# rishihahs/pupperv3-mjx

Hardware: AMD Instinct MI355X
Metric: env-steps/sec at N_envs=4096/GPU, 1/2/4/8 MI355X; qpos rel-err vs mj_step (higher is better)
Workload: dtype f32

## Files before the change

### pupperv3-mjx_amd/csrc/pp3_env.hip

```cpp
#include <hip/hip_runtime.h>

#include <float.h>
#include <math.h>
#include <stddef.h>
#include <stdio.h>
#include <stdlib.h>
#include <string.h>

#include <string>
#include <algorithm>
#include <vector>

#include "pp3_device.h"
#include "pp3_diag.h"
#include "pp3_mlp.h"

namespace pp3 {

constexpr int HW = 32;
typedef __attribute__((address_space(4))) const DevModel GModel;
typedef __attribute__((address_space(4))) const float GFloat;
constexpr int HMAX = 16;
constexpr int OBS_MOVE = (PP3_OBS_DIM * (HMAX - 1) + HW - 1) / HW;
template <int HCAP, int LAGCAP>
// ... 580 lines not shown
  if (r >= c) { r -= c; m >>= 8; pos += 8; }
  c = __popc(m & 0xFu);
  if (r >= c) { r -= c; m >>= 4; pos += 4; }
  c = __popc(m & 0x3u);
  if (r >= c) { r -= c; m >>= 2; pos += 2; }
  return pos + (r >= (int)(m & 1u) ? 1 : 0);
}

template <int NC, int NWV = 1, bool CULL = false>
__device__ __forceinline__ int collision(Shared<NC>& s, const DevModel& m, int l, int h, const PairLoad& pre,
                                         float* ccache = nullptr) {
  int nhit = 0;
  const TerrainRef tr{m.terrain, m.nbox};
  auto run = [&](int p, const PairLoad& pl) {
    float dist = 0, pos[3], nrm[3];
    v4f pc0;
    const bool hit = narrow<NC, NWV>(s, tr, pl, dist, pos, nrm, pc0) && p >= 0;
    const uint32_t mask = hballot(hit, h);
    const int slot = nhit + __popc(mask & ((1u << l) - 1u));
    if (hit) {
      if (slot < NC) store_contact(s, pc0, slot, p, dist, pos, nrm);
      if (slot < NHIT) { s.x.a.hit_dist[slot] = dist; s.x.a.hit_pair[slot] = p; }
    }
    nhit += __popc(mask);
  };
  if (!CULL || !m.cull_on) {
    for (int base = 0; base < m.npair; base += HW) {
      const int p = base + l;
      float dist = 0, pos[3], nrm[3];
      v4f pc0;
      const PairLoad pl = base == 0 ? pre : load_pair(m, p < m.npair ? p : 0);
      const bool hit = narrow<NC, NWV>(s, tr, pl, dist, pos, nrm, pc0) && (p < m.npair);
      const uint32_t mask = hballot(hit, h);
      const int slot = nhit + __popc(mask & ((1u << l) - 1u));
      if (hit) {
        if (slot < NC) store_contact(s, pc0, slot, p, dist, pos, nrm);
        if (slot < NHIT) { s.x.a.hit_dist[slot] = dist; s.x.a.hit_pair[slot] = p; }
      }
      nhit += __popc(mask);
    }
  } else {
    const uint32_t pbox = m.pair_box4[l];
    const float b0 = s.xpos[1][0], b1 = s.xpos[1][1], b2 = s.xpos[1][2];
    {
      const float c0 = b0 - ccache[0], c1 = b1 - ccache[1], c2 = b2 - ccache[2];
      const bool stale = !(c0 * c0 + c1 * c1 + c2 * c2 <= CULL_SLACK * CULL_SLACK);
      if (__ballot(stale)) {
        const int b = l < tr.nbox ? l : 0;
        v4f bx[4];
        if (tr.terrain) {
          typedef __attribute__((address_space(1))) const v4f GF4;
          const int env_raw = 2 * NWV * blockIdx.x + (threadIdx.x >> 5);
          const GF4* t = (const GF4*)(uintptr_t)tr.terrain + ((size_t)env_raw * tr.nbox + b) * 4;
#pragma unroll
          for (int k = 0; k < 4; k++) bx[k] = t[k];
        } else {
#pragma unroll
          for (int k = 0; k < 4; k++) bx[k] = reinterpret_cast<const v4f*>(&m.box_tab[b])[k];
        }
        const float reach = m.cull_reach + CULL_SLACK;
        const float d0 = b0 - bx[0][0], d1 = b1 - bx[0][1], d2 = b2 - bx[0][2];
        const float R[9] = {bx[0][3], bx[1][0], bx[1][1], bx[1][2], bx[1][3], bx[2][0], bx[2][1], bx[2][2], bx[2][3]};
        bool far = false;
#pragma unroll
        for (int k = 0; k < 3; k++) far |= fabsf(R[k] * d0 + R[3 + k] * d1 + R[6 + k] * d2) > bx[3][k] + reach;
        const uint32_t nm = hballot(l < tr.nbox && !far, h);
        if (l == 0) {
          ccache[0] = b0;
          ccache[1] = b1;
          ccache[2] = b2;
          ccache[3] = __uint_as_float(nm);
        }
        SYNC();
      }
    }
    const uint32_t near = __float_as_uint(ccache[3]);
    uint32_t cm[4];
    int total = 0;
#pragma unroll
    for (int k = 0; k < 4; k++) {
      const int p = 32 * (k + 1) + l;
      const uint32_t bs = (pbox >> (8 * k)) & 0xFFu;
      const bool c = p < m.npair && (bs >= 32u || ((near >> (bs & 31u)) & 1u));
      cm[k] = hballot(c, h);
      total += __popc(cm[k]);
    }
    const int rounds = wmax2(total);
    auto cand = [&](int base) {
      int p = -1, r = base + l;
#pragma unroll
      for (int k = 0; k < 4; k++) {
        const int c = __popc(cm[k]);
        if (p < 0 && r < c) p = 32 * (k + 1) + nth_bit(cm[k], r);
        if (p < 0) r -= c;
      }
      return p;
    };
    const int p1 = cand(0);
    const PairLoad pl1 = load_pair(m, p1 >= 0 ? p1 : 0);
    run(l < m.npair ? l : -1, pre);
    if (rounds > 0) run(p1, pl1);
    for (int base = HW; base < rounds; base += HW) {
      const int p = cand(base);
      run(p, load_pair(m, p >= 0 ? p : 0));
    }
  }
  if (l == 0) { s.nhit = nhit; s.ncon = nhit < NC ? nhit : NC; }
  const bool ovf = nhit > NC;
  if (__ballot(ovf)) {
    SYNC();
    const int nh = nhit < NHIT ? nhit : NHIT;
    int keep_p[NHIT / HW];
    bool keep[NHIT / HW];
    int rank[NHIT / HW];
#pragma unroll
    for (int t = 0; t < NHIT / HW; t++) {
      const int i = l + HW * t;
      const float myd = i < nh ? s.x.a.hit_dist[i] : 0.0f;
      int r = 0;
      for (int c = 0; c < nh; c++) {
        const float dc = s.x.a.hit_dist[c];
        r += (dc < myd || (dc == myd && c < i)) ? 1 : 0;
      }
      rank[t] = r;
      keep[t] = ovf && i < nh && r < NC;
      keep_p[t] = i < nh ? s.x.a.hit_pair[i] : 0;
    }
    int before = 0;
    int slot[NHIT / HW];
#pragma unroll
    for (int t = 0; t < NHIT / HW; t++) {
      const uint32_t km = hballot(keep[t], h);
      slot[t] = before + __popc(km & ((1u << l) - 1u));
      before += __popc(km);
    }
    (void)rank;
    SYNC();
#pragma unroll
    for (int t = 0; t < NHIT / HW; t++) {
      if (keep[t]) {
        float dist, pos[3], nrm[3];
        v4f pc0;
        narrow<NC, NWV>(s, tr, load_pair(m, keep_p[t]), dist, pos, nrm, pc0);
        store_contact(s, pc0, slot[t], keep_p[t], dist, pos, nrm);
      }
    }
  }
  SYNC();
  const int ncon_h = nhit < NC ? nhit : NC;
  const int sup = s.con_sup[l < NC ? l : 0];
  return l < ncon_h ? sup : 4;
}

template <int NC>
__device__ __forceinline__ void rne_chain(Shared<NC>& s, const DevModel& m, int l) {
  if (l >= 4) return;
  float lcd[3][6], lqd[3];
#pragma unroll
  for (int k = 0; k < 3; k++) {
    const int d = 6 + 3 * l + k;
#pragma unroll
    for (int c = 0; c < 6; c++) lcd[k][c] = s.cdof[d][c];
    lqd[k] = s.qvel[d];
  }
  PIN("+v"(lcd[0][0]), "+v"(lcd[0][1]), "+v"(lcd[0][2]), "+v"(lcd[0][3]), "+v"(lcd[0][4]), "+v"(lcd[0][5]),
      "+v"(lcd[1][0]), "+v"(lcd[1][1]), "+v"(lcd[1][2]), "+v"(lcd[1][3]), "+v"(lcd[1][4]), "+v"(lcd[1][5]),
      "+v"(lcd[2][0]), "+v"(lcd[2][1]), "+v"(lcd[2][2]), "+v"(lcd[2][3]), "+v"(lcd[2][4]), "+v"(lcd[2][5]),
      "+v"(lqd[0]), "+v"(lqd[1]), "+v"(lqd[2]));
  float bcd[3][6], bq[6];
#pragma unroll
  for (int d = 0; d < 3; d++)
#pragma unroll
    for (int k = 0; k < 6; k++) bcd[d][k] = s.cdof[3 + d][k];
#pragma unroll
  for (int k = 0; k < 6; k++) bq[k] = s.qvel[k];
  PIN("+v"(bcd[0][0]), "+v"(bcd[0][1]), "+v"(bcd[0][2]), "+v"(bcd[0][3]), "+v"(bcd[0][4]), "+v"(bcd[0][5]),
      "+v"(bcd[1][0]), "+v"(bcd[1][1]), "+v"(bcd[1][2]), "+v"(bcd[1][3]), "+v"(bcd[1][4]), "+v"(bcd[1][5]),
      "+v"(bcd[2][0]), "+v"(bcd[2][1]), "+v"(bcd[2][2]), "+v"(bcd[2][3]), "+v"(bcd[2][4]), "+v"(bcd[2][5]),
      "+v"(bq[0]), "+v"(bq[1]), "+v"(bq[2]), "+v"(bq[3]), "+v"(bq[4]), "+v"(bq[5]));
  float w[3] = {0, 0, 0}, bsum[3] = {0, 0, 0};
#pragma unroll
  for (int d = 0; d < 3; d++) {
    const float q = bq[3 + d];
#pragma unroll
    for (int k = 0; k < 3; k++) { w[k] += bcd[d][k] * q; bsum[k] += bcd[d][3 + k] * q; }
  }
  const float v0 = bq[0], v1 = bq[1], v2 = bq[2];
  float cv[6] = {w[0], w[1], w[2], v0 + bsum[0], v1 + bsum[1], v2 + bsum[2]};
  float ca[6] = {0, 0, 0, -m.gravity[0] + (v1 * w[2] - v2 * w[1]), -m.gravity[1] + (v2 * w[0] - v0 * w[2]),
                 -m.gravity[2] + (v0 * w[1] - v1 * w[0])};
  float cdd[6];
  if (l == 0)
    for (int k = 0; k < 6; k++) { s.cvel[1][k] = cv[k]; s.x.a.cacc[1][k] = ca[k]; }
#pragma unroll
  for (int k = 0; k < 3; k++) {
    const int b = 2 + 3 * l + k;
    cross_motion(cdd, cv, lcd[k]);
    const float qd = lqd[k];
    for (int c = 0; c < 6; c++) { cv[c] += lcd[k][c] * qd; ca[c] += cdd[c] * qd; }
    for (int c = 0; c < 6; c++) { s.cvel[b][c] = cv[c]; s.x.a.cacc[b][c] = ca[c]; }
  }
}

template <int NC>
__device__ __forceinline__ void rne_body_forces(Shared<NC>& s, int l, int h) {
  float cf[6] = {0, 0, 0, 0, 0, 0};
  if (l >= 1 && l < NB) {
    float f1[6], f2[6], f3[6];
    mul_inert_vec(f1, s.cinert[l], s.x.a.cacc[l]);
    mul_inert_vec(f2, s.cinert[l], s.cvel[l]);
    cross_force(f3, s.cvel[l], f2);
    for (int k = 0; k < 6; k++) { cf[k] = f1[k] + f3[k]; s.x.a.cacc[l][k] = cf[k]; }
  }
  float t[6];
#pragma unroll
  for (int k = 0; k < 6; k++) t[k] = hsum_lane16(cf[k]);
  if (l == 16)
#pragma unroll
    for (int k = 0; k < 6; k++) s.cfrc_base[k] = t[k];
}

template <int NC>
__device__ __forceinline__ void crb_times_cdof(Shared<NC>& s, const DevModel& m, int l) {
  if (l >= NV) return;
  const bool base = l < 6;
  const int b = base ? 2 : l - 4, last = 2 + 3 * ((b - 2) / 3) + 2;
  const float* r0 = base ? s.crb_base : s.cinert[b];
  const int b1 = b + 1 <= last ? b + 1 : b, b2 = b + 2 <= last ? b + 2 : b;
  float crb[10], c1[10], c2[10], cdv[6];
#pragma unroll
  for (int k = 0; k < 10; k++) { crb[k] = r0[k]; c1[k] = s.cinert[b1][k]; c2[k] = s.cinert[b2][k]; }
#pragma unroll
  for (int k = 0; k < 6; k++) cdv[k] = s.cdof[l][k];
  PIN("+v"(crb[0]), "+v"(crb[1]), "+v"(crb[2]), "+v"(crb[3]), "+v"(crb[4]), "+v"(crb[5]), "+v"(crb[6]), "+v"(crb[7]),
      "+v"(crb[8]), "+v"(crb[9]), "+v"(cdv[0]), "+v"(cdv[1]), "+v"(cdv[2]), "+v"(cdv[3]), "+v"(cdv[4]), "+v"(cdv[5]));
  PIN("+v"(c1[0]), "+v"(c1[1]), "+v"(c1[2]), "+v"(c1[3]), "+v"(c1[4]), "+v"(c1[5]), "+v"(c1[6]), "+v"(c1[7]),
      "+v"(c1[8]), "+v"(c1[9]), "+v"(c2[0]), "+v"(c2[1]), "+v"(c2[2]), "+v"(c2[3]), "+v"(c2[4]), "+v"(c2[5]),
      "+v"(c2[6]), "+v"(c2[7]), "+v"(c2[8]), "+v"(c2[9]));
  const float w1 = (!base && b + 1 <= last) ? 1.0f : 0.0f, w2 = (!base && b + 2 <= last) ? 1.0f : 0.0f;
#pragma unroll
  for (int k = 0; k < 10; k++) crb[k] += w1 * c1[k];
#pragma unroll
  for (int k = 0; k < 10; k++) crb[k] += w2 * c2[k];
  mul_inert_vec(s.x.a.F[l], crb, cdv);
}


__device__ __forceinline__ int opaque_lane(int l) {
  asm volatile("" : "+v"(l));
  __builtin_assume(l >= 0 && l < HW);
  return l;
}

__device__ __forceinline__ void ldl_rows(float (&a)[NV], float& dinv, int l, float* col) {
  l = opaque_lane(l);
  const int slot = l < NV ? l : NV;
#pragma unroll
  for (int k = 0; k < NV; ++k) {
    col[slot] = a[k];
    SYNC();
    float r[20];
#pragma unroll
    for (int q = (k & ~3); q < 20; q += 4) {
      const float4 v = *reinterpret_cast<const float4*>(col + q);
      r[q] = v.x; r[q + 1] = v.y; r[q + 2] = v.z; r[q + 3] = v.w;
    }
    const float ik = frcp(fmaxf(r[k], MINVAL));
    dinv = (l == k) ? ik : dinv;
    const float lik = a[k] * ik;
#pragma unroll
    for (int j = k + 1; j < NV; ++j) a[j] -= lik * r[j];
    a[k] = (l > k) ? lik : a[k];
    SYNC();
  }
}
template <int NC>
__device__ __forceinline__ float ldl_solve(Shared<NC>& s, const float (&a)[NV], float dinv, float x, int l, int h) {
  l = opaque_lane(l);
  const int li = l < NV ? l : NV - 1;
#pragma unroll
  for (int k = 0; k < NV; ++k)
    if (k < l && l < NV) s.x.L[l][k] = a[k];
#pragma unroll
  for (int k = 0; k < NV - 1; ++k) {
    const float yk = hb(x, k, h);
    x = (l > k) ? x - a[k] * yk : x;
  }
  x = x * dinv;
  SYNC();
  float col[NV];
#pragma unroll
  for (int k = 1; k < NV; ++k) col[k] = s.x.L[k][li];
#pragma unroll
  for (int k = NV - 1; k > 0; --k) {
    const float xk = hb(x, k, h);
    x = (l < k) ? x - col[k] * xk : x;
  }
  return x;
}

__host__ __device__ constexpr int pnat(int p) { return p < 12 ? p + 6 : p - 12; }
__host__ __device__ constexpr int npos(int d) { return d < 6 ? d + 12 : d - 6; }

__device__ __forceinline__ float dpp_shl1(float v) { return dpp_f<0x101, 0xF>(v, 0.0f); }
__device__ __forceinline__ float dpp_shl2(float v) { return dpp_f<0x102, 0xF>(v, 0.0f); }

// ... 280 lines not shown
    const int o = 6 + 3 * (sup & 3);
    v2f jj[9];
    float xv[K][9];
    float x1[K];
#pragma unroll
    for (int i = 0; i < 9; i++) {
      const int col = i < 6 ? i : o + i - 6;
      jj[i] = v2f{s.Jc[c][0][col], s.Jc[c][t][col]};
#pragma unroll
      for (int k = 0; k < K; k++) xv[k][i] = xs[k][col];
    }
#pragma unroll
    for (int k = 0; k < K; k++) x1[k] = xs[k][col1];
    if constexpr (K == 1) {
      PIN("+v"(jj[0]), "+v"(jj[1]), "+v"(jj[2]), "+v"(jj[3]), "+v"(jj[4]), "+v"(jj[5]), "+v"(jj[6]), "+v"(jj[7]),
          "+v"(jj[8]), "+v"(xv[0][0]), "+v"(xv[0][1]), "+v"(xv[0][2]), "+v"(xv[0][3]), "+v"(xv[0][4]),
          "+v"(xv[0][5]), "+v"(xv[0][6]), "+v"(xv[0][7]), "+v"(xv[0][8]), "+v"(x1[0]));
    } else {
      static_assert(K == 2 || K == 3, "row_dotk: K = 1, 2 or 3");
      PIN("+v"(jj[0]), "+v"(jj[1]), "+v"(jj[2]), "+v"(jj[3]), "+v"(jj[4]), "+v"(jj[5]), "+v"(jj[6]), "+v"(jj[7]),
          "+v"(jj[8]), "+v"(xv[0][0]), "+v"(xv[0][1]), "+v"(xv[0][2]), "+v"(xv[0][3]), "+v"(xv[0][4]),
          "+v"(xv[0][5]), "+v"(xv[0][6]), "+v"(xv[0][7]), "+v"(xv[0][8]), "+v"(xv[1][0]), "+v"(xv[1][1]),
          "+v"(xv[1][2]), "+v"(xv[1][3]), "+v"(xv[1][4]), "+v"(xv[1][5]), "+v"(xv[1][6]), "+v"(xv[1][7]),
          "+v"(xv[1][8]), "+v"(x1[0]), "+v"(x1[1]));
      if constexpr (K == 3)
        PIN("+v"(xv[2][0]), "+v"(xv[2][1]), "+v"(xv[2][2]), "+v"(xv[2][3]), "+v"(xv[2][4]), "+v"(xv[2][5]),
            "+v"(xv[2][6]), "+v"(xv[2][7]), "+v"(xv[2][8]), "+v"(x1[2]));
    }
#pragma unroll
    for (int i = 0; i < 9; i++)
#pragma unroll
      for (int k = 0; k < K; k++) { a[k] += jj[i].x * xv[k][i]; b[k] += jj[i].y * xv[k][i]; }
#pragma unroll
    for (int k = 0; k < K; k++) out[k] = (isf || isl) ? sg1 * x1[k] : a[k] + sg * mu * b[k];
    return;
  }
#pragma unroll
  for (int k = 0; k < K; k++) out[k] = (isf || isl) ? sg1 * xs[k][col1] : a[k] + sg * mu * b[k];
}
template <int NC>
__device__ __forceinline__ float row_dot(const Shared<NC>& s, int r, int nl, int ncon, const float* x) {
  const float* const xs[1] = {x};
  float o[1];
  row_dotk<NC, 1>(s, r, nl, ncon, xs, o);
  return o[0];
}

template <int J0, int J1>
__device__ __forceinline__ void hess_acc(float (&a)[NV], const float (&J)[3][NV], float w0, float w1, float w2) {
#pragma unroll
  for (int j = J0; j < J1; j++) a[j] = fmaf(w2, J[2][j], fmaf(w1, J[1][j], fmaf(w0, J[0][j], a[j])));
}

template <int LAGCAP = PP3_MAX_LAG>
__device__ __forceinline__ int choice_from_uniform(const GFloat* dist, int n, float u) {
  float d[LAGCAP];
#pragma unroll
  for (int i = 0; i < LAGCAP; i++) d[i] = dist[i];
  float total = 0.0f;
#pragma unroll
  for (int i = 0; i < LAGCAP; i++)
    if (i < n) total += d[i];
  const float r = total * (1.0f - u);
  float acc = 0.0f;
  int li = 0;
#pragma unroll
  for (int i = 0; i < LAGCAP; i++)
    if (i < n) {
      acc += d[i];
      li += (acc < r) ? 1 : 0;
    }
  return li < n ? li : n - 1;
}

template <int NC>
using LdsShared = __attribute__((address_space(3))) Shared<NC>;
template <int NC>
__device__ __attribute__((noinline)) void dense_search(LdsShared<NC>* sp, int l, int h, int cmax, int ncon, int lsup) {
  Shared<NC>& s = *(Shared<NC>*)sp;
  {
    const bool ll = (lsup & 7) == 5;
    const bool known = (lsup & 8) != 0;
    const int p = (lsup >> 4) & 3, q = (lsup >> 6) & 3;
    const uint64_t bll = __ballot(ll), bunk = __ballot(ll && !known);
    uint64_t bl[4];
#pragma unroll
    for (int g = 0; g < 4; g++) bl[g] = __ballot(ll && known && (p == g || q == g));
    int lbh[2];
    bool okh[2];
#pragma unroll
    for (int hh = 0; hh < 2; hh++) {
      const uint64_t hm = hh ? 0xFFFFFFFF00000000ull : 0xFFFFFFFFull;
      const int n = __popcll(bll & hm);
      int b = 0;
      bool found = false;
#pragma unroll
      for (int g = 3; g >= 0; g--)
        if (__popcll(bl[g] & hm) == n) { b = g; found = true; }
      okh[hh] = found && (bunk & hm) == 0;
      lbh[hh] = b;
    }
    if (okh[0] && okh[1]) {
      const int lb = h ? lbh[1] : lbh[0];
      const int lp = l < NV ? l : NV - 1, dn = pnat(lp);
      float a[NV];
#pragma unroll
      for (int j = 0; j < NV; j++) a[j] = s.M[dn][pnat(j)];
      const float dD = s.dofD[dn];
#pragma unroll
      for (int j = 0; j < NV; j++) a[j] += (j == lp) ? dD : 0.0f;
      for (int c = 0; c < cmax; c++) {
        const int sa = __builtin_amdgcn_readlane(lsup, c), sb = __builtin_amdgcn_readlane(lsup, HW + c);
        if (c < ncon) {
          const float* G = s.con_G[c];
          const float jn = s.Jc[c][0][dn], j1 = s.Jc[c][1][dn], j2 = s.Jc[c][2][dn];
          const float w0 = jn * G[0] + j1 * G[1] + j2 * G[2];
          const float w1 = jn * G[1] + j1 * G[3];
          const float w2 = jn * G[2] + j2 * G[4];
          const bool any = (sa & 7) == 5 || (sb & 7) == 5;
          hess_acc_p<0, 6>(a, s.Jc[c], w0, w1, w2);
          if (any || sa == 0 || sb == 0) hess_acc_p<6, 9>(a, s.Jc[c], w0, w1, w2);
          if (any || sa == 1 || sb == 1) hess_acc_p<9, 12>(a, s.Jc[c], w0, w1, w2);
          if (any || sa == 2 || sb == 2) hess_acc_p<12, 15>(a, s.Jc[c], w0, w1, w2);
          if (any || sa == 3 || sb == 3) hess_acc_p<15, 18>(a, s.Jc[c], w0, w1, w2);
        }
      }
      const float x = ldl_arrow_solve_b(a, s.grad[dn], l, &s.x.L[0][0], lb);
      if (l < NV) s.search[dn] = -x;
      return;
    }
  }
  const int li = l < NV ? l : NV - 1;
  float a[NV], dinv = 1.0f;
#pragma unroll
  for (int j = 0; j < NV; j++) a[j] = s.M[li][j];
  const float dD = s.dofD[li];
#pragma unroll
  for (int j = 0; j < NV; j++) a[j] += (j == li) ? dD : 0.0f;
  for (int c = 0; c < cmax; c++) {
    if (c < ncon) {
      const float* G = s.con_G[c];
      const float jn = s.Jc[c][0][li], j1 = s.Jc[c][1][li], j2 = s.Jc[c][2][li];
      const float w0 = jn * G[0] + j1 * G[1] + j2 * G[2];
      const float w1 = jn * G[1] + j1 * G[3];
      const float w2 = jn * G[2] + j2 * G[4];
      hess_acc<0, NV>(a, s.Jc[c], w0, w1, w2);
    }
  }
  ldl_rows(a, dinv, l, &s.x.L[0][0]);
  const float x = ldl_solve(s, a, dinv, s.grad[li], l, h);
  if (l < NV) s.search[l] = -x;
}

template <int NC, int NWV = 1, bool LIBSC = true, bool CULL = false>
__device__ __forceinline__ int substep(Shared<NC>& s, const DevModel& m, int l, int h, bool integrate_prev,
                                       const KinConst& kc PROF_PARAM, float* ccache = nullptr) {
  constexpr int NR = (Shared<NC>::NEFC + HW - 1) / HW;
  l = opaque_lane(l);
  LaneRec<2> rc_pf;
  LaneRec<3> rm_pf;
  {
    v4f v[5];
#pragma unroll
    for (int k = 0; k < 2; k++) v[k] = *reinterpret_cast<const v4f*>(at_bytes(m.lane_com, 16u * (unsigned)l) + k * 128);
#pragma unroll
    for (int k = 0; k < 2; k++)
      for (int c = 0; c < 4; c++) rc_pf.f[4 * k + c] = v[k][c];
#pragma unroll
    for (int k = 0; k < 3; k++) v[2 + k] = *reinterpret_cast<const v4f*>(at_bytes(m.lane_m, 16u * (unsigned)l) + k * 128);
#pragma unroll
    for (int k = 0; k < 3; k++)
      for (int c = 0; c < 4; c++) rm_pf.f[4 * k + c] = v[2 + k][c];
  }
  kinematics<NC, LIBSC>(s, m, l, integrate_prev, kc); SYNC();
  PHASE(0); l = opaque_lane(l);
  { com_pos(s, m, l, h, rc_pf); SYNC(); }
  PHASE(1); l = opaque_lane(l);
  const PairLoad pair_pf = load_pair(m, l < m.npair ? l : 0);
  { crb_times_cdof(s, m, l); rne_chain(s, m, l); SYNC(); }
  PHASE(15); l = opaque_lane(l);
  int lsup = 4;
  { lsup = collision<NC, NWV, CULL>(s, m, l, h, pair_pf, ccache); SYNC(); }
  PHASE(16); l = opaque_lane(l);
  v4f pcv[4];
  {
    const LaneRec<7> rl = fetch_rec(m.lane_lim, l);
    const int jlim = l < 2 * (NJ - 1) ? 1 + (l >> 1) : 1;
    const bool actl = l < NU;
    const int adof = actl ? as_i(rl.f[LL_ACT_DOF]) : 0, aqadr = actl ? as_i(rl.f[LL_ACT_QADR]) : 0;
    float lq = s.qpos[7 + jlim - 1], lqv = s.qvel[6 + jlim - 1], fqv = s.qvel[6 + (l < NFR ? l : 0)];
    float actrl = s.ctrl[actl ? l : 0], aq = s.qpos[aqadr], aqv = s.qvel[adof];
    float skp = s.kp, skd = s.kd;
    int sdr = s.dr_on;
    PIN("+v"(lq), "+v"(lqv), "+v"(fqv), "+v"(actrl), "+v"(aq), "+v"(aqv), "+v"(skp), "+v"(skd), "+v"(sdr));
    bool act = false;
    float value = 0;
    int j = 0;
    if (l < 2 * (NJ - 1)) {
      j = 1 + (l >> 1);
      const float side = (l & 1) ? 1.0f : -1.0f;
      if (as_i(rl.f[LL_LIM_ON])) {
        value = side * (rl.f[LL_RANGE] - lq);
        act = value < rl.f[LL_MARGIN];
      }
    }
    const uint32_t mask = hballot(act, h);
    const int slot = __popc(mask & ((1u << l) - 1u));
    const int nlb = __popc(mask) < NLMAX ? __popc(mask) : NLMAX;
    if (act && slot < NLMAX) {
      const int dof = 6 + j - 1;
      const float sg = (l & 1) ? -1.0f : 1.0f;
      s.lim_dof[slot] = dof;
      s.lim_sgn[slot] = sg;
      const float imp = getimp(&rl.f[LL_SOLIMP], value, rl.f[LL_MARGIN]);
      const float R = fmaxf(MINVAL, (1.0f - imp) / imp * rl.f[LL_INVW]);
      const int r = NFR + slot;
      s.efc_R[r] = R;
      s.efc_D[r] = 1.0f / R;
      s.efc_aref[r] = -rl.f[LL_B] * (sg * lqv) - rl.f[LL_K] * imp * (value - rl.f[LL_MARGIN]);
      (void)dof;
    }
    if (l == 0) s.nl = nlb;
    if (l < NFR) {
      const int dof = 6 + l;
      s.efc_R[l] = rl.f[LL_FR_R];
      s.efc_D[l] = 1.0f / rl.f[LL_FR_R];
      s.efc_aref[l] = -rl.f[LL_FR_B] * fqv;
      (void)dof;
    }
    if (l < NU) {
      const int d = adof, flags = as_i(rl.f[LL_ACT_FLAGS]);
      float ctrl = actrl;
      if (flags & ACTF_CTRLLIMITED) ctrl = fminf(fmaxf(ctrl, rl.f[LL_CRANGE]), rl.f[LL_CRANGE + 1]);
      const float gear = rl.f[LL_GEAR];
      const float len = gear * aq, vel = gear * aqv;
      float gain = rl.f[LL_GAIN], b0 = rl.f[LL_BIAS], b1 = rl.f[LL_BIAS + 1], b2 = rl.f[LL_BIAS + 2];
      if (sdr) { gain = skp; b1 = -skp; b2 = -skd; }
      float force = gain * ctrl;
      if (flags & ACTF_AFFINE) force += b0 + b1 * len + b2 * vel;
      if (flags & ACTF_FORCELIMITED) force = fminf(fmaxf(force, rl.f[LL_FRANGE]), rl.f[LL_FRANGE + 1]);
      s.qfrc_act[d] = gear * force;
    }
    if (l < 6) s.qfrc_act[l] = 0.0f;
    {
      const int pe = l - NFR - nlb, pcon = pe >> 2;
      const int p = (pe >= 0 && pcon < s.ncon) ? s.con_pair[(pe >= 0 && pcon < NC) ? pcon : 0] : 0;
      const GV4* src = pair_con_groups(m, p);
#pragma unroll
      for (int k = 0; k < 4; k++) pcv[k] = src[k];
    }
  }
  SYNC();
  PHASE(2); l = opaque_lane(l);
  const LaneRec<3> rm = rm_pf;
  
  constexpr int NT = (NMPAIR + HW - 1) / HW;
  float cd[NT][6], fi[NT][6];
#pragma unroll
  for (int t = 0; t < NT; t++) {
    const int ij = as_i(rm.f[LM_IJ + t]);
    const int i = ij < 0 ? 0 : (ij & 0xff), j = ij < 0 ? 0 : (ij >> 8);
#pragma unroll
    for (int k = 0; k < 6; k++) { cd[t][k] = s.cdof[j][k]; fi[t][k] = s.x.a.F[i][k]; }
  }
#pragma unroll
  for (int t = 0; t < NT; t++)
    PIN("+v"(cd[t][0]), "+v"(cd[t][1]), "+v"(cd[t][2]), "+v"(cd[t][3]), "+v"(cd[t][4]), "+v"(cd[t][5]),
        "+v"(fi[t][0]), "+v"(fi[t][1]), "+v"(fi[t][2]), "+v"(fi[t][3]), "+v"(fi[t][4]), "+v"(fi[t][5]));
#pragma unroll
  for (int t = 0; t < NT; t++) {
    const int ij = as_i(rm.f[LM_IJ + t]);
    if (ij < 0) continue;
    const int i = ij & 0xff, j = ij >> 8;
    float v = 0;
#pragma unroll
    for (int k = 0; k < 6; k++) v += cd[t][k] * fi[t][k];
    v += rm.f[LM_ARM + t];
    s.M[i][j] = v;
    s.M[j][i] = v;
  }
  rne_body_forces(s, l, h);
  const int ncon = s.ncon;
  __builtin_assume(ncon >= 0 && ncon <= NC);
  for (int it = l; it < ncon * NV; it += HW) {
    const int c = it / NV, i = it - c * NV;
    const uint32_t bit = 1u << i;
    float cp[3], cm[3], cd[6], fr[9];
    uint32_t dm0 = s.con_dm[c][0], dm1 = s.con_dm[c][1];
#pragma unroll
    for (int k = 0; k < 3; k++) { cp[k] = s.x.a.con_pos[c][k]; cm[k] = s.com[k]; }
#pragma unroll
    for (int k = 0; k < 6; k++) cd[k] = s.cdof[i][k];
#pragma unroll
    for (int k = 0; k < 9; k++) fr[k] = s.x.a.con_frame[c][k];
    PIN("+v"(cp[0]), "+v"(cp[1]), "+v"(cp[2]), "+v"(cm[0]), "+v"(cm[1]), "+v"(cm[2]), "+v"(cd[0]), "+v"(cd[1]),
        "+v"(cd[2]), "+v"(cd[3]), "+v"(cd[4]), "+v"(cd[5]), "+v"(fr[0]), "+v"(fr[1]), "+v"(fr[2]), "+v"(fr[3]),
        "+v"(fr[4]), "+v"(fr[5]), "+v"(fr[6]), "+v"(fr[7]), "+v"(fr[8]), "+v"(dm0), "+v"(dm1));
    const float off[3] = {cp[0] - cm[0], cp[1] - cm[1], cp[2] - cm[2]};
    float cr[3], jp[3];
    cross3(cr, cd, off);
    const float w = ((dm1 & bit) ? 1.0f : 0.0f) - ((dm0 & bit) ? 1.0f : 0.0f);
    for (int k = 0; k < 3; k++) jp[k] = w * (cd[3 + k] + cr[k]);
    s.Jc[c][0][i] = fr[0] * jp[0] + fr[1] * jp[1] + fr[2] * jp[2];
    s.Jc[c][1][i] = fr[3] * jp[0] + fr[4] * jp[1] + fr[5] * jp[2];
    s.Jc[c][2][i] = fr[6] * jp[0] + fr[7] * jp[1] + fr[8] * jp[2];
  }
  SYNC();
  PHASE(3); l = opaque_lane(l);
  {
  if (l < NV) {
    const bool base = l < 6;
    const int b = base ? 2 : l - 4, last = 2 + 3 * ((b - 2) / 3) + 2;
    const int b1 = b + 1 <= last ? b + 1 : b, b2 = b + 2 <= last ? b + 2 : b;
    float r0[6], c0[6], c1[6], c2[6], cdv[6];
#pragma unroll
    for (int k = 0; k < 6; k++) {
      r0[k] = s.cfrc_base[k];
      c0[k] = s.x.a.cacc[b][k];
      c1[k] = s.x.a.cacc[b1][k];
      c2[k] = s.x.a.cacc[b2][k];
      cdv[k] = s.cdof[l][k];
    }
    float qv = s.qvel[l], qa = s.qfrc_act[l];
    PIN("+v"(r0[0]), "+v"(r0[1]), "+v"(r0[2]), "+v"(r0[3]), "+v"(r0[4]), "+v"(r0[5]), "+v"(c0[0]), "+v"(c0[1]),
        "+v"(c0[2]), "+v"(c0[3]), "+v"(c0[4]), "+v"(c0[5]), "+v"(cdv[0]), "+v"(cdv[1]), "+v"(cdv[2]), "+v"(cdv[3]),
        "+v"(cdv[4]), "+v"(cdv[5]), "+v"(qv), "+v"(qa));
    PIN("+v"(c1[0]), "+v"(c1[1]), "+v"(c1[2]), "+v"(c1[3]), "+v"(c1[4]), "+v"(c1[5]), "+v"(c2[0]), "+v"(c2[1]),
        "+v"(c2[2]), "+v"(c2[3]), "+v"(c2[4]), "+v"(c2[5]));
    const float w1 = b + 1 <= last ? 1.0f : 0.0f, w2 = b + 2 <= last ? 1.0f : 0.0f;
    float cf[6];
#pragma unroll
    for (int k = 0; k < 6; k++) {
      float t = c0[k];
      t += w1 * c1[k];
      t += w2 * c2[k];
      cf[k] = base ? r0[k] : t;
    }
    float bias = 0;
    for (int k = 0; k < 6; k++) bias += cdv[k] * cf[k];
    s.qfrc_smooth[l] = -rm.f[LM_DAMP] * qv - bias + qa;
  }
  }
  const int nl = s.nl;
  __builtin_assume(nl >= 0 && nl <= NLMAX);
  const int nefc = NFR + nl + 4 * ncon;
  SYNC();
  PHASE(13); l = opaque_lane(l);
  float mrow[NV];
  {
    const int lp = l < NV ? l : NV - 1, dn = pnat(lp);
    float a[NV];
#pragma unroll
    for (int j = 0; j < NV; j++) { a[j] = s.M[dn][pnat(j)]; mrow[j] = a[j]; }
    const float x = ldl_arrow_solve(a, s.qfrc_smooth[dn], l, &s.x.L[0][0]);
    s.qacc_smooth[dn] = x;
  }
  SYNC();
  PHASE(4); l = opaque_lane(l);

  float Dr[NR], Rr[NR], ar[NR], fl[NR];
  bool valid[NR], isfr[NR];
#pragma unroll
  for (int t = 0; t < NR; t++) {
    const int r = l + HW * t;
    valid[t] = r < nefc;
    isfr[t] = r < NFR;
    Dr[t] = valid[t] ? s.efc_D[r] : 0.0f;
    Rr[t] = valid[t] ? s.efc_R[r] : 0.0f;
    ar[t] = valid[t] ? s.efc_aref[r] : 0.0f;
    fl[t] = (valid[t] && isfr[t]) ? rm.f[LM_FLOSS] : 0.0f;
  }
  float cws = 0, csm = 0;
  float xws[NR], xsm[NR], ma_ws = 0.0f;
  bool use_smooth;
  {
#pragma unroll
    for (int t = 0; t < NR; t++) {
      xws[t] = 0.0f;
      xsm[t] = 0.0f;
      if (!valid[t]) continue;
      const int r = l + HW * t;
      const int e0 = r - NFR - nl, cc = e0 < 0 ? 0 : ((e0 >> 2) < NC ? (e0 >> 2) : NC - 1);
      float cb = 0.0f, cp = 0.0f;
      if (e0 >= 0) {
        const float mu = s.con_mu[cc];
        const float dist = s.con_dist[cc];
        LaneRec<4> pc;
        if (t == 0) {
#pragma unroll
          for (int k = 0; k < 4; k++)
#pragma unroll
            for (int c4 = 0; c4 < 4; c4++) pc.f[4 * k + c4] = pcv[k][c4];
        } else {
          pc = fetch_rec(*reinterpret_cast<const LaneRec<4>*>(&m.pair_con[s.con_pair[cc]]));
        }
        const PairCon& q = *reinterpret_cast<const PairCon*>(&pc);
        const float tran = q.tran;
        const float invw = (tran + mu * mu * tran) * 2.0f * mu * mu / m.impratio;
        const float imp = getimp(q.solimp, dist, q.margin);
        const float R = fmaxf(MINVAL, (1.0f - imp) / imp * invw);
        Rr[t] = R;
        Dr[t] = 1.0f / R;
        cb = q.b;
        cp = q.k * imp * (dist - q.margin);
      }
      const float* const xs[3] = {s.qws, s.qacc_smooth, s.qvel};
      float d[3];
      row_dotk<NC, 3>(s, r, nl, ncon, xs, d);
      ar[t] = e0 >= 0 ? -cb * d[2] - cp : ar[t];
      const float d1 = d[0], d2 = d[1];
      const float x1 = d1 - ar[t];
      const float x2 = d2 - ar[t];
      xws[t] = x1;
      xsm[t] = x2;
      const float rf = Rr[t] * fl[t];
      const float q1 = 0.5f * Dr[t] * x1 * x1, q2 = 0.5f * Dr[t] * x2 * x2;
      const float f1 = (x1 <= -rf) ? (-fl[t] * x1 - 0.5f * rf * fl[t]) : (x1 >= rf) ? (fl[t] * x1 - 0.5f * rf * fl[t]) : q1;
      const float f2 = (x2 <= -rf) ? (-fl[t] * x2 - 0.5f * rf * fl[t]) : (x2 >= rf) ? (fl[t] * x2 - 0.5f * rf * fl[t]) : q2;
      cws += isfr[t] ? f1 : ((x1 < 0) ? q1 : 0.0f);
      csm += isfr[t] ? f2 : ((x2 < 0) ? q2 : 0.0f);
    }
    PHASE(23);
    if (l < NV) {
      const int dn = pnat(l);
      ma_ws = mrow_dot_reg(mrow, s.qws);
      cws += 0.5f * (ma_ws - s.qfrc_smooth[dn]) * (s.qws[dn] - s.qacc_smooth[dn]);
    }
    cws = hsum(cws, h);
    csm = hsum(csm, h);
    use_smooth = cws > csm;
    {
      const int lc = l < NV ? l : NV - 1;
      s.qacc[lc] = use_smooth ? s.qacc_smooth[lc] : s.qws[lc];
    }
// ... 765 lines not shown
  const StepArgs* ap_step;
  if constexpr (NWV > 1) ap_step = (const StepArgs*)ap;
  else ap_step = FUSED ? (const StepArgs*)ap : &a_arg;
  const StepArgs& a = *ap_step;
  if constexpr (NWV > 1) {
    typedef __attribute__((address_space(4))) const PolicyStepArgs GPArgs;
    const GPArgs& pa = *(const GPArgs*)ap;
    const int Hm = ((const DevModel*)(const GModel*)a.m)->H;
    const bool tile_in = PP3_OBS_DIM * Hm + 4 <= OBS_TILE_W;
    if (tile_in && it == 0) {
      for (int i = threadIdx.x; i < pp3pol::TILE * PP3_OBS_DIM * Hm; i += WAVE * NWV) {
        const int r = i / (PP3_OBS_DIM * Hm), k = i - r * (PP3_OBS_DIM * Hm);
        const int row = blockIdx.x * pp3pol::TILE + r;
        obs_tile[r][k] = row < a.N ? a.obs_out[(size_t)row * (PP3_OBS_DIM * Hm) + k] : 0.0f;
      }
    }
    __syncthreads();
    PP3_STEP_ACQUIRE();
    if constexpr (SAMPLE) {
      policy_mlp_sample((GSArgs*)ap, tile_in ? (LdsObsTile*)obs_tile : (LdsObsTile*)nullptr, it, Hm,
                        ((const DevModel*)(const GModel*)a.m)->partitionable,
                        (pp3pol::LdsTileBuf*)(reinterpret_cast<pp3pol::TileBuf*>(sh)),
                        (LdsU32*)&obs_tile[pp3pol::TILE][0]);
      PP3_STEP_ACQUIRE();
    } else {
      if (tile_in)
        policy_mlp_tile(&pa.net, pa.act + (size_t)it * a.act_stride, a.N, blockIdx.x * pp3pol::TILE,
                        (pp3pol::LdsTileBuf*)(reinterpret_cast<pp3pol::TileBuf*>(sh)), (LdsObsTile*)obs_tile);
      else
        policy_mlp(&pa.net, a.obs_out, PP3_OBS_DIM * Hm, pa.act + (size_t)it * a.act_stride, a.N,
                   blockIdx.x * pp3pol::TILE, (pp3pol::LdsTileBuf*)(reinterpret_cast<pp3pol::TileBuf*>(sh)));
      PP3_STEP_ACQUIRE();
    }
  }
  int lane = NWV > 1 ? (int)(threadIdx.x & (WAVE - 1)) : (int)threadIdx.x;
  if (FUSED) asm volatile("" : "+v"(lane));
  const int wv = NWV > 1 ? __builtin_amdgcn_readfirstlane(threadIdx.x >> 6) : 0;
  const int h = lane >> 5, l = lane & (HW - 1);
  Shared<NC>& s = sh[alias ? 0 : 2 * wv + h];
  const int env_raw = 2 * (blockIdx.x * NWV + wv) + h;
  const bool own = env_raw < a.N;
  const int env = own ? env_raw : a.N - 1;
  const GModel* mp_pro = (const GModel*)(a.m);
  if (FUSED) asm volatile("" : "+s"(mp_pro));
  const DevModel& m = *(const DevModel*)mp_pro;
  const int stride = m.stride;
  const int part = m.partitionable;
  float* gst = a.state + (size_t)env * stride;
  float* const to = TG && a.traj_obs ? a.traj_obs + ((size_t)it * a.N + env) * (PP3_OBS_DIM * m.H) : nullptr;
  int n_frames = __builtin_amdgcn_readfirstlane(m.n_frames);
  const float* act_env = a.actions + (size_t)it * a.act_stride + (size_t)env * NU;
  const size_t obs_base = (size_t)env * (PP3_OBS_DIM * m.H);
  const float* oi = a.obs_in + obs_base;
  float* oo = a.obs_out + obs_base;
  const bool carry = FUSED && NWV == 1 && it > 0;
  float arow[CAPS::LAG], irow[CAPS::LAG], act_in = 0.0f;
  {
    const float* ar = gst + PP3_S_ACT_BUF + (l < NU ? l : 0) * m.La;
    const float* ir = gst + m.imu_off + (l < 6 ? l : 0) * m.Li;
#pragma unroll
    for (int q = 0; q < CAPS::LAG; q++) {
      arow[q] = (l < NU && q < m.La) ? ar[q] : 0.0f;
      irow[q] = (l < 6 && q < m.Li) ? ir[q] : 0.0f;
    }
    if (l < NU) act_in = act_env[l];
  }
  LaneRec<2> re;
  for (int k = 0; k < 2; k++)
    for (int c = 0; c < 4; c++) re.f[4 * k + c] = m.lane_env.g[k][l][c];
  const KinConst kc = kin_const(m, l);
  const int nmove = PP3_OBS_DIM * (m.H - 1);
  const bool hist_lds = carry && nmove == PP3_OBS_DIM;
  float tmp[CAPS::MOVE > 0 ? CAPS::MOVE : 1];
#pragma unroll
  for (int t = 0; t < CAPS::MOVE; t++) {
    const int k = l + HW * t;
    if (hist_lds) tmp[t] = (k < PP3_OBS_DIM) ? s.x.e.o[k < PP3_OBS_DIM ? k : 0] : 0.0f;
    else tmp[t] = (k < nmove) ? oi[k] : 0.0f;
  }
  float v[(PP3_S_ACT_BUF + HW - 1) / HW];
  if (!carry)
#pragma unroll
    for (int t = 0; t < (PP3_S_ACT_BUF + HW - 1) / HW; t++) v[t] = l + HW * t < PP3_S_ACT_BUF ? gst[l + HW * t] : 0.0f;
  if (a.episode) {
    if (l == 0) {
      s.ep_prev_done = a.done[env];
      s.ep_racc = a.phase > 0 ? a.reward[env] : 0.0f;
    }
    if (l < PP3_EP_STRIDE) s.ep[l] = a.episode[(size_t)env * PP3_EP_STRIDE + l];
  }
  if (!carry) load_params(s, m, a.dr ? a.dr + (size_t)env * PP3_NDR : nullptr, l);
  if (!hist_lds) asm volatile("s_waitcnt vmcnt(0)" ::: "memory");
  if (own)
#pragma unroll
    for (int t = 0; t < CAPS::MOVE; t++)
      if (l + HW * t < nmove) {
        oo[PP3_OBS_DIM + l + HW * t] = tmp[t];
        if constexpr (NWV > 1)
          if (PP3_OBS_DIM * m.H + 4 <= OBS_TILE_W) obs_tile[2 * wv + h][PP3_OBS_DIM + l + HW * t] = tmp[t];
        if (TG && to) to[PP3_OBS_DIM + l + HW * t] = tmp[t];
      }
  if (!carry)
#pragma unroll
    for (int t = 0; t < (PP3_S_ACT_BUF + HW - 1) / HW; t++)
      if (l + HW * t < PP3_S_ACT_BUF) s.st[l + HW * t] = v[t];
  SYNC();
  if (l < NQ) s.qpos[l] = s.st[PP3_S_QPOS + l];
  if (l < NV) { s.qvel[l] = s.st[PP3_S_QVEL + l]; s.qws[l] = s.st[PP3_S_QACC_WS + l]; }
  const Key rng{__float_as_uint(s.st[PP3_S_RNG]), __float_as_uint(s.st[PP3_S_RNG + 1])};
  const Key kl = split_i(rng, 5, l < 5 ? l : 0, part);
  const Key k_new = hkey(kl, 0, h), cmd_key = hkey(kl, 1, h);
  const Key kkick = hkey(kl, 2, h), kbern = hkey(kl, 3, h), klat = hkey(kl, 4, h);
  float u = 0;
  if (l < 4) {
    const Key kk = l < 2 ? kkick : (l == 2 ? kbern : klat);
    u = uniform_i(kk, l < 2 ? 2 : 1, l < 2 ? l : 0, l < 2 ? -1.0f : 0.0f, 1.0f, part);
  }
  const float bern = hb(u, 2, h) < m.kick_p ? 1.0f : 0.0f;
  const float kick0 = hb(u, 0, h) * m.kick_vel * bern, kick1 = hb(u, 1, h) * m.kick_vel * bern;
  const int li = choice_from_uniform<CAPS::LAG>((const GFloat*)m.lat_dist, m.La, hb(u, 3, h));
  if (l == 0) {
    s.qvel[0] += kick0;
    s.qvel[1] += kick1;
    s.st[PP3_S_KICK] = kick0;
    s.st[PP3_S_KICK + 1] = kick1;
    s.st[PP3_S_RNG] = __uint_as_float(k_new.a);
    s.st[PP3_S_RNG + 1] = __uint_as_float(k_new.b);
  }
  if (l < NU) {
    const float lagged = push_lagged_pre<CAPS::LAG>(gst + PP3_S_ACT_BUF + l * m.La, m.La, act_in, li, own, arow);
    const float t = re.f[LE_POSE] + lagged * m.action_scale;
    s.ctrl[l] = fminf(fmaxf(t, re.f[LE_JLO]), re.f[LE_JHI]);
  }
  SYNC();
  float* imu_stash = s.st + PP3_S_QPOS;
  if (l < 6)
#pragma unroll
    for (int q = 0; q < CAPS::LAG; q++) imu_stash[PP3_MAX_LAG * l + q] = irow[q];
  SYNC();
  PHASE(10);
  asm volatile("" : "+s"(n_frames));
  uint32_t hwid;
  asm volatile("s_getreg_b32 %0, hwreg(HW_REG_HW_ID)" : "=s"(hwid));
  const int wslot = (int)(hwid & 1u);
  int heavy = heavy_prev;
  for (int f = 0; f < n_frames; f++) {
    const int prio = 2 * heavy + ((f + wslot) & 1);
    if (prio == 3) __builtin_amdgcn_s_setprio(3);
    else if (prio == 2) __builtin_amdgcn_s_setprio(2);
    else if (prio == 1) __builtin_amdgcn_s_setprio(1);
    else __builtin_amdgcn_s_setprio(0);
    const GModel* mp = (const GModel*)(a.m);
    asm volatile("" : "+s"(mp));
    const int wgt = substep<NC, NWV, FUSED, CULL>(s, *(const DevModel*)mp, l, h, f > 0, kc PROF_ARG,
                                                  CULL ? cull_cache[alias ? 0 : 2 * wv + h] : nullptr);
    heavy = wgt >= HEAVY_WEIGHT ? 1 : 0;
  }
  if (n_frames > 0) {
    const GModel* mp = (const GModel*)(a.m);
    asm volatile("" : "+s"(mp));
    euler_step<NC, FUSED>(s, *(const DevModel*)mp, l);
    PHASE(9);
  }
  if (heavy) __builtin_amdgcn_s_setprio(3);
  else if (wslot) __builtin_amdgcn_s_setprio(1);
  else __builtin_amdgcn_s_setprio(0);
  SYNC();
  const GModel* mq = (const GModel*)(a.m);
  asm volatile("" : "+s"(mq));
  {
  const DevModel& m = *(const DevModel*)mq;
  const LaneRec<2> re = fetch_rec(m.lane_env, l);
  get_obs<NC, CAPS::LAG>(s, m, gst + m.imu_off, l, h, re.f[LE_POSE16], own, imu_stash PROF_ARG);
  {
    if (own)
      for (int k = l; k < PP3_OBS_DIM; k += HW) {
        oo[k] = s.x.e.o[k];
        if constexpr (NWV > 1)
          if (PP3_OBS_DIM * m.H + 4 <= OBS_TILE_W) obs_tile[2 * wv + h][k] = s.x.e.o[k];
        if (TG && to) to[k] = s.x.e.o[k];
      }
  }
  SYNC();
  if (l < NQ) s.st[PP3_S_QPOS + l] = s.qpos[l];
  if (l < NV) { s.st[PP3_S_QVEL + l] = s.qvel[l]; s.st[PP3_S_QACC_WS + l] = s.qws[l]; }
  SYNC();
  PHASE(11);
  const int tb = m.torso_body;
  const int bx = (l >= 1 && l < NB) ? l : 1, fx = (l >= 16 && l < 20) ? l - 16 : 0;
  float xbb[3], cm[3], cv[6], qt[4];
#pragma unroll
  for (int k = 0; k < 3; k++) { xbb[k] = s.xpos[bx][k]; cm[k] = s.com[k]; }
#pragma unroll
  for (int k = 0; k < 6; k++) cv[k] = s.cvel[bx][k];
#pragma unroll
  for (int k = 0; k < 4; k++) qt[k] = s.xquat[tb][k];
  float fz = s.foot_xpos[fx][2], lcst = s.st[PP3_S_LAST_CONTACT + fx], airt0 = s.st[PP3_S_AIR_TIME + fx];
  float xtz = s.xpos[tb][2], qpl = s.qpos[7 + (l < 12 ? l : 0)];
  float cmd0 = s.st[PP3_S_COMMAND], cmd1 = s.st[PP3_S_COMMAND + 1], cmd2 = s.st[PP3_S_COMMAND + 2];
  PIN("+v"(xbb[0]), "+v"(xbb[1]), "+v"(xbb[2]), "+v"(cm[0]), "+v"(cm[1]), "+v"(cm[2]), "+v"(cv[0]), "+v"(cv[1]),
      "+v"(cv[2]), "+v"(cv[3]), "+v"(cv[4]), "+v"(cv[5]), "+v"(qt[0]), "+v"(qt[1]), "+v"(qt[2]), "+v"(qt[3]));
  PIN("+v"(fz), "+v"(lcst), "+v"(airt0), "+v"(xtz), "+v"(qpl), "+v"(cmd0), "+v"(cmd1), "+v"(cmd2));
  if (l >= 1 && l < NB) {
    const int b = l;
    const float off[3] = {xbb[0] - cm[0], xbb[1] - cm[1], xbb[2] - cm[2]};
    float cr[3];
    cross3(cr, cv, off);
    for (int k = 0; k < 3; k++) { s.x.e.xdv[b][k] = cv[3 + k] + cr[k]; s.x.e.xda[b][k] = cv[k]; }
  }
  if (l >= 16 && l < 20) {
    const int f = l - 16;
    const float cz = fz - m.foot_radius;
    const int last = lcst != 0.0f;
    const int c = cz < 1e-3f;
    s.x.e.contact[f] = c;
    s.x.e.filt_mm[f] = c | last;
    s.x.e.filt_cm[f] = (cz < 3e-2f) | last;
    s.x.e.first[f] = (airt0 > 0.0f && (c | last)) ? 1.0f : 0.0f;
    s.st[PP3_S_AIR_TIME + f] = airt0 + m.dt;
  }
  SYNC();
  const float z0[3] = {0, 0, 1};
  float ru_t[3];
  b_rotate(ru_t, z0, qt);
  const bool jviol = l < 12 && (qpl < re.f[LE_JLO] || qpl > re.f[LE_JHI]);
  const bool isdone = hballot(jviol, h) != 0 || ru_t[2] < m.cos_term_angle || xtz < m.term_z;
  const float cn = sqrtf(cmd0 * cmd0 + cmd1 * cmd1 + cmd2 * cmd2);
  float r_torq = 0, r_jacc = 0, r_mech = 0, r_arate = 0, r_stand = 0, r_standv = 0, r_abd = 0;
  float r_air = 0, r_slip = 0, r_knee = 0, r_body = 0;
  const int l18 = l < NV ? l : 0, l12 = l < 12 ? l : 0, l4 = l < 4 ? l : 0, lc = l < NC ? l : 0;
  const int bleg = l < 4 ? as_i(re.f[LE_LEG]) : 1;
  float fa = s.qfrc_act[l18], fa6 = s.qfrc_act[6 + l12], qv = s.qvel[6 + l12], qp = s.qpos[7 + l12];
  float lvel = s.st[PP3_S_LAST_VEL + l12], lact = s.st[PP3_S_LAST_ACT + l12];
  float airt = s.st[PP3_S_AIR_TIME + l4], fst = s.x.e.first[l4];
  float sp[3], xb[3], xdab[3], xdvb[2];
#pragma unroll
  for (int k = 0; k < 3; k++) { sp[k] = s.foot_xpos[l4][k]; xb[k] = s.xpos[bleg][k]; xdab[k] = s.x.e.xda[bleg][k]; }
  xdvb[0] = s.x.e.xdv[bleg][0];
  xdvb[1] = s.x.e.xdv[bleg][1];
  int fcm = s.x.e.filt_cm[l4], ncon_r = s.ncon, cpair = s.con_pair[lc];
  float cdist = s.con_dist[lc];
  PIN("+v"(fa), "+v"(fa6), "+v"(qv), "+v"(qp), "+v"(lvel), "+v"(lact), "+v"(airt), "+v"(fst), "+v"(sp[0]), "+v"(sp[1]),
      "+v"(sp[2]), "+v"(xb[0]), "+v"(xb[1]), "+v"(xb[2]), "+v"(xdab[0]), "+v"(xdab[1]), "+v"(xdab[2]), "+v"(xdvb[0]),
      "+v"(xdvb[1]), "+v"(fcm), "+v"(ncon_r), "+v"(cpair), "+v"(cdist));
  if (l < NV) r_torq = fa * fa;
  if (l < 12) {
    const float acc = (qv - lvel) / m.env_dt;
    r_jacc = acc * acc;
    r_mech = fabsf(fa6 * qv);
    const float da = act_in - lact;
    r_arate = da * da;
    r_stand = fabsf(qp - re.f[LE_POSE]);
    r_standv = fabsf(qv);
    if (l % 3 == 1) { const float t = qp - re.f[LE_ABD]; r_abd = t * t; }
  }
  if (l < 4) {
    r_air = (airt - 0.1f) * fst;
    const float off[3] = {sp[0] - xb[0], sp[1] - xb[1], sp[2] - xb[2]};
    float cr[3];
    cross3(cr, xdab, off);
    const float vx = xdvb[0] + cr[0], vy = xdvb[1] + cr[1];
    r_slip = (vx * vx + vy * vy) * (fcm ? 1.0f : 0.0f);
  }
  if (l < ncon_r && cdist < 0.0f) {
    const v4f kb = pair_con_groups(m, cpair)[3];
    r_knee = kb[1];
    r_body = kb[2];
  }
  r_torq = hsum(r_torq, h);
  r_jacc = hsum(r_jacc, h);
  r_mech = hsum(r_mech, h);
  r_arate = hsum(r_arate, h);
  r_stand = hsum(r_stand, h) * ((cn < 0.1f) ? 1.0f : 0.0f);
  r_standv = hsum(r_standv, h) * ((cn < m.stand_thr) ? 1.0f : 0.0f);
  r_abd = hsum(r_abd, h);
  r_air = hsum(r_air, h) * ((cn > 0.05f) ? 1.0f : 0.0f);
  r_slip = hsum(r_slip, h);
  r_knee = hsum(r_knee, h);
  r_body = hsum(r_body, h);
  float rw[PP3_NREWARD];
  {
    const float inv[4] = {s.xquat[1][0], -s.xquat[1][1], -s.xquat[1][2], -s.xquat[1][3]};
    const float sig = m.sigma;
    const float* xdv1 = s.x.e.xdv[1];
    const float* xda1 = s.x.e.xda[1];
    float lv[3], av[3], wz[3], ru[3];
    b_rotate(lv, xdv1, inv);
    b_rotate(av, xda1, inv);
    b_rotate(wz, z0, inv);
    b_rotate(ru, z0, s.xquat[1]);
    const float e_lin = (cmd0 - lv[0]) * (cmd0 - lv[0]) + (cmd1 - lv[1]) * (cmd1 - lv[1]);
    float e_ori = 0;
    for (int k = 0; k < 3; k++) e_ori += (wz[k] - s.st[PP3_S_DESIRED_Z + k]) * (wz[k] - s.st[PP3_S_DESIRED_Z + k]);
    rw[PP3_REWARD_TRACKING_LIN_VEL] = expf(-e_lin / sig);
    rw[PP3_REWARD_TRACKING_ANG_VEL] = expf(-(cmd2 - av[2]) * (cmd2 - av[2]) / sig);
    rw[PP3_REWARD_TRACKING_ORIENTATION] = expf(-e_ori / sig);
    rw[PP3_REWARD_LIN_VEL_Z] = xdv1[2] * xdv1[2];
    rw[PP3_REWARD_ANG_VEL_XY] = xda1[0] * xda1[0] + xda1[1] * xda1[1];
    rw[PP3_REWARD_ORIENTATION] = ru[0] * ru[0] + ru[1] * ru[1];
  }
  rw[PP3_REWARD_TORQUES] = r_torq;
  rw[PP3_REWARD_JOINT_ACCELERATION] = r_jacc;
  rw[PP3_REWARD_MECHANICAL_WORK] = r_mech;
  rw[PP3_REWARD_ACTION_RATE] = r_arate;
  rw[PP3_REWARD_STAND_STILL] = r_stand;
  rw[PP3_REWARD_STAND_STILL_JOINT_VELOCITY] = r_standv;
  rw[PP3_REWARD_ABDUCTION_ANGLE] = r_abd;
// ... 1619 lines not shown
```

Measured before the change: 55.74 million.

## Parallelize RNE velocity/acceleration recursion across body lanes using DPP shifts

Replaces the per-leg serial RNE chain (4 lanes) plus a separate body-force pass with a per-body-lane formulation. Each lane computes its body's velocity and acceleration by propagating parent values through DPP row shifts across the three chain levels, then computes body forces and a 16-lane reduction of base force in the same phase. The aim is to spread the recursion over more lanes and drop the later rne_body_forces pass. The legacy path is kept for one template configuration (NC==16 with CULL and not FUSED). This relies on lane ordering matching the kinematic tree layout.

```diff
diff --git a/pupperv3-mjx_amd/csrc/pp3_env.hip b/pupperv3-mjx_amd/csrc/pp3_env.hip
--- a/pupperv3-mjx_amd/csrc/pp3_env.hip
+++ b/pupperv3-mjx_amd/csrc/pp3_env.hip
@@ -756,6 +756,98 @@
   return l < ncon_h ? sup : 4;
 }
 
+__device__ __forceinline__ float dpp_shr1(float v) {
+  return __int_as_float(__builtin_amdgcn_update_dpp(0, __float_as_int(v), 0x111, 0xF, 0xF, true));
+}
+
+template <int NC>
+__device__ __forceinline__ void rne_bodies(Shared<NC>& s, const DevModel& m, int l) {
+  const bool body = l >= 1 && l < NB;
+  const int b = body ? l : 1;
+  const int lev = b >= 2 ? (b - 2) % 3 : -1;
+  const int dj = b >= 2 ? 4 + b : 6;
+  float lcd[6], lqd = s.qvel[dj], ci[10];
+#pragma unroll
+  for (int c = 0; c < 6; c++) lcd[c] = s.cdof[dj][c];
+#pragma unroll
+  for (int c = 0; c < 10; c++) ci[c] = s.cinert[b][c];
+  float bcd[3][6], bq[6];
+#pragma unroll
+  for (int d = 0; d < 3; d++)
+#pragma unroll
+    for (int k = 0; k < 6; k++) bcd[d][k] = s.cdof[3 + d][k];
+#pragma unroll
+  for (int k = 0; k < 6; k++) bq[k] = s.qvel[k];
+  unsigned goff = (unsigned)(reinterpret_cast<const char*>(m.gravity) - reinterpret_cast<const char*>(&m));
+  asm volatile("" : "+v"(goff));
+  const float* gp = at_bytes(m, goff);
+  float g0 = gp[0], g1 = gp[1], g2 = gp[2];
+  PIN("+v"(g0), "+v"(g1), "+v"(g2));
+  PIN("+v"(lcd[0]), "+v"(lcd[1]), "+v"(lcd[2]), "+v"(lcd[3]), "+v"(lcd[4]), "+v"(lcd[5]), "+v"(lqd), "+v"(ci[0]),
+      "+v"(ci[1]), "+v"(ci[2]), "+v"(ci[3]), "+v"(ci[4]), "+v"(ci[5]), "+v"(ci[6]), "+v"(ci[7]), "+v"(ci[8]), "+v"(ci[9]));
+  PIN("+v"(bcd[0][0]), "+v"(bcd[0][1]), "+v"(bcd[0][2]), "+v"(bcd[0][3]), "+v"(bcd[0][4]), "+v"(bcd[0][5]),
+      "+v"(bcd[1][0]), "+v"(bcd[1][1]), "+v"(bcd[1][2]), "+v"(bcd[1][3]), "+v"(bcd[1][4]), "+v"(bcd[1][5]),
+      "+v"(bcd[2][0]), "+v"(bcd[2][1]), "+v"(bcd[2][2]), "+v"(bcd[2][3]), "+v"(bcd[2][4]), "+v"(bcd[2][5]),
+      "+v"(bq[0]), "+v"(bq[1]), "+v"(bq[2]), "+v"(bq[3]), "+v"(bq[4]), "+v"(bq[5]));
+  float w[3] = {0, 0, 0}, bsum[3] = {0, 0, 0};
+#pragma unroll
+  for (int d = 0; d < 3; d++) {
+    const float q = bq[3 + d];
+#pragma unroll
+    for (int k = 0; k < 3; k++) { w[k] += bcd[d][k] * q; bsum[k] += bcd[d][3 + k] * q; }
+  }
+  const float v0 = bq[0], v1 = bq[1], v2 = bq[2];
+  const float cvb[6] = {w[0], w[1], w[2], v0 + bsum[0], v1 + bsum[1], v2 + bsum[2]};
+  const float cab[6] = {0, 0, 0, -g0 + (v1 * w[2] - v2 * w[1]), -g1 + (v2 * w[0] - v0 * w[2]),
+                        -g2 + (v0 * w[1] - v1 * w[0])};
+  float cv[6], ca[6];
+  {
+    float cdd[6];
+    cross_motion(cdd, cvb, lcd);
+#pragma unroll
+    for (int c = 0; c < 6; c++) {
+      const float tv = cvb[c] + lcd[c] * lqd, ta = cab[c] + cdd[c] * lqd;
+      cv[c] = lev >= 0 ? tv : cvb[c];
+      ca[c] = lev >= 0 ? ta : cab[c];
+    }
+  }
+#pragma unroll
+  for (int lv = 1; lv < 3; lv++) {
+    float pv[6], pa[6], cdd[6];
+    PIN("+v"(cv[0]), "+v"(cv[1]), "+v"(cv[2]), "+v"(cv[3]), "+v"(cv[4]), "+v"(cv[5]), "+v"(ca[0]), "+v"(ca[1]),
+        "+v"(ca[2]), "+v"(ca[3]), "+v"(ca[4]), "+v"(ca[5]));
+#pragma unroll
+    for (int c = 0; c < 6; c++) { pv[c] = dpp_shr1(cv[c]); pa[c] = dpp_shr1(ca[c]); }
+    PIN("+v"(pv[0]), "+v"(pv[1]), "+v"(pv[2]), "+v"(pv[3]), "+v"(pv[4]), "+v"(pv[5]), "+v"(pa[0]), "+v"(pa[1]),
+        "+v"(pa[2]), "+v"(pa[3]), "+v"(pa[4]), "+v"(pa[5]));
+    cross_motion(cdd, pv, lcd);
+#pragma unroll
+    for (int c = 0; c < 6; c++) {
+      const float tv = pv[c] + lcd[c] * lqd, ta = pa[c] + cdd[c] * lqd;
+      cv[c] = lev >= lv ? tv : cv[c];
+      ca[c] = lev >= lv ? ta : ca[c];
+    }
+  }
+  float cf[6];
+  {
+    float f1[6], f2[6], f3[6];
+    mul_inert_vec(f1, ci, ca);
+    mul_inert_vec(f2, ci, cv);
+    cross_force(f3, cv, f2);
+#pragma unroll
+    for (int k = 0; k < 6; k++) cf[k] = body ? f1[k] + f3[k] : 0.0f;
+  }
+  if (body)
+#pragma unroll
+    for (int k = 0; k < 6; k++) { s.cvel[b][k] = cv[k]; s.x.a.cacc[b][k] = cf[k]; }
+  float t[6];
+#pragma unroll
+  for (int k = 0; k < 6; k++) t[k] = hsum_lane16(cf[k]);
+  if (l == 16)
+#pragma unroll
+    for (int k = 0; k < 6; k++) s.cfrc_base[k] = t[k];
+}
+
 template <int NC>
 __device__ __forceinline__ void rne_chain(Shared<NC>& s, const DevModel& m, int l) {
   if (l >= 4) return;
@@ -1342,7 +1434,7 @@
   if (l < NV) s.search[l] = -x;
 }
 
-template <int NC, int NWV = 1, bool LIBSC = true, bool CULL = false>
+template <int NC, int NWV = 1, bool LIBSC = true, bool CULL = false, bool LEGRNE = false>
 __device__ __forceinline__ int substep(Shared<NC>& s, const DevModel& m, int l, int h, bool integrate_prev,
                                        const KinConst& kc PROF_PARAM, float* ccache = nullptr) {
   constexpr int NR = (Shared<NC>::NEFC + HW - 1) / HW;
@@ -1367,7 +1459,11 @@
   { com_pos(s, m, l, h, rc_pf); SYNC(); }
   PHASE(1); l = opaque_lane(l);
   const PairLoad pair_pf = load_pair(m, l < m.npair ? l : 0);
-  { crb_times_cdof(s, m, l); rne_chain(s, m, l); SYNC(); }
+  {
+    crb_times_cdof(s, m, l);
+    if constexpr (LEGRNE) rne_chain(s, m, l); else rne_bodies(s, m, l);
+    SYNC();
+  }
   PHASE(15); l = opaque_lane(l);
   int lsup = 4;
   { lsup = collision<NC, NWV, CULL>(s, m, l, h, pair_pf, ccache); SYNC(); }
@@ -1469,7 +1565,7 @@
     s.M[i][j] = v;
     s.M[j][i] = v;
   }
-  rne_body_forces(s, l, h);
+  if constexpr (LEGRNE) rne_body_forces(s, l, h);
   const int ncon = s.ncon;
   __builtin_assume(ncon >= 0 && ncon <= NC);
   for (int it = l; it < ncon * NV; it += HW) {
@@ -2541,7 +2637,7 @@
     else __builtin_amdgcn_s_setprio(0);
     const GModel* mp = (const GModel*)(a.m);
     asm volatile("" : "+s"(mp));
-    const int wgt = substep<NC, NWV, FUSED, CULL>(s, *(const DevModel*)mp, l, h, f > 0, kc PROF_ARG,
+    const int wgt = substep<NC, NWV, FUSED, CULL, NC == 16 && CULL && !FUSED>(s, *(const DevModel*)mp, l, h, f > 0, kc PROF_ARG,
                                                   CULL ? cull_cache[alias ? 0 : 2 * wv + h] : nullptr);
     heavy = wgt >= HEAVY_WEIGHT ? 1 : 0;
   }
```

New measurement: 56.54 million, median of 6. 1.01x the previous value.
